# facebookresearch/pytorchvideo

Measured on NVIDIA H100. Metric: clips/sec forward (synthetic 3xTx224^2), higher is better.
Workload: dtype f16

## Files before the change

### include/pv_b200.h

```cpp
#ifndef PV_B200_H_
#define PV_B200_H_

#include <stdint.h>

#ifdef __cplusplus
extern "C" {
#endif

#define PV_ABI_VERSION 1

typedef enum pv_status {
  PV_OK = 0,
  PV_ERR_INVALID = -1,
  PV_ERR_CUDA = -2,
  PV_ERR_UNSUPPORTED = -3,
  PV_ERR_NO_DEVICE = -4
} pv_status;

typedef enum pv_dtype { PV_F16 = 0, PV_F32 = 1, PV_U8 = 2, PV_I64 = 3  } pv_dtype;

typedef enum pv_act {
  PV_ACT_NONE = 0,
  PV_ACT_RELU = 1,
  PV_ACT_SWISH = 2,
  PV_ACT_GELU = 3,
  PV_ACT_SIGMOID = 4,
  PV_ACT_HSWISH = 5
} pv_act;

typedef enum pv_conv_algo {
  PV_ALGO_AUTO = 0,
  PV_ALGO_DIRECT = 1,
  PV_ALGO_TCGEN05 = 2
} pv_conv_algo;

typedef enum pv_pool_mode { PV_POOL_MAX = 0, PV_POOL_AVG = 1 } pv_pool_mode;

int pv_abi_version(void);
const char* pv_last_error(void);
int pv_device_info(int* sm_count, int* cc);
long long pv_launch_count(void);
int pv_kernel_counts(char* buf, int len);

typedef struct pv_clip_transform_desc {
  int C, n_t, out_h, out_w;
  long long sc, st, sh, sw;
  float mean[4], stdv[4];
  int src_dtype;
  int dst_dtype;
  int div255;
} pv_clip_transform_desc;

int pv_clip_transform_fwd(const pv_clip_transform_desc* d, const void* src,
                          const int32_t* idx_t,
                          const int32_t* y0, const int32_t* y1, const float* ly,
                          const int32_t* x0, const int32_t* x1, const float* lx,
                          void* dst, void* stream);

typedef struct pv_clip_batch_desc {
  int C, n_clips, n_t, n_slow;
  int in_h, in_w, new_h, new_w;
  int top, left, out_h, out_w;
  int hflip;
  long long sc, st, sh, sw, s_clip;
  long long d_clip, d_slow_clip;
  float mean[4], stdv[4];
  int div255, normalize;
  int src_dtype, dst_dtype;
} pv_clip_batch_desc;

int pv_clip_transform_batch(const pv_clip_batch_desc* d, const void* src, const int32_t* idx_t,
                            const int32_t* slow_pos, const int32_t* geom, void* dst, void* dst_slow,
                            void* stream);

int pv_clip_transform_rrc(const pv_clip_batch_desc* d, const void* src, const int32_t* idx_t, const int32_t* boxes,
                          void* dst, void* stream);

#define PV_BOX_F32 1
#define PV_BOX_F64 3
#define PV_BOX_CLIP_SRC 1
#define PV_BOX_SCALE 2
#define PV_BOX_CROP 4
#define PV_BOX_CLIP_CROP 8
#define PV_BOX_FLIP 16
#define PV_BOX_CLIP_OUT 32
#define PV_BOX_ALL_STEPS 63

typedef struct pv_boxes_desc {
  int n_clips, n_boxes;
  int steps;
  int dtype;
  int in_h, in_w;
  int new_h, new_w, top, left, hflip;
  int out_h, out_w;
} pv_boxes_desc;

int pv_clip_boxes_transform(const pv_boxes_desc* d, const void* boxes_in, const int32_t* box_start,
                            const int32_t* geom, void* boxes_out, float* rois_out, void* stream);

typedef enum pv_aug_kind {
  PV_AUG_NONE = 0, PV_AUG_BRIGHTNESS = 1, PV_AUG_CONTRAST = 2, PV_AUG_SATURATION = 3, PV_AUG_SHARPNESS = 4,
  PV_AUG_AUTOCONTRAST = 5, PV_AUG_EQUALIZE = 6, PV_AUG_INVERT = 7, PV_AUG_POSTERIZE = 8, PV_AUG_SOLARIZE = 9,
  PV_AUG_AFFINE = 10
} pv_aug_kind;

typedef struct pv_aug_op {
  int kind;
  int ival;
  float ratio;
  float omr;
  float theta[6];
  float fill[3];
} pv_aug_op;

typedef struct pv_aug_frame_stats {
  float mn[3], mx[3];
  double gray_sum;
  unsigned char lut[3][256];
} pv_aug_frame_stats;

typedef struct pv_augment_desc {
  int n_clips, src_div, T, C, H, W;
  long long s_clip, st, sc, sh, sw;
  int dtype;
} pv_augment_desc;

int pv_augment_stats(const pv_augment_desc* d, const void* src, pv_aug_frame_stats* stats, void* stream);
int pv_augment_apply(const pv_augment_desc* d, const void* src, const pv_aug_op* ops, const pv_aug_frame_stats* stats,
                     void* dst, void* stream);
int pv_augment_mix(const pv_augment_desc* d, const void* src, const void* chains, int width, const float* mix,
                   void* dst, void* stream);

typedef struct pv_mix_desc {
  int B;
  int dtype;
  long long size[4];
  long long stride[4];
  long long s_batch;
} pv_mix_desc;

typedef struct pv_mix_label_desc {
  int B, K;
  int one_hot;
  int mode;
  float lam, oml;
  float on, off;
  long long s_row, s_col;
} pv_mix_label_desc;

int pv_mixup(const pv_mix_desc* d, void* x, float lam, float oml, void* stream);
int pv_cutmix(const pv_mix_desc* d, void* x, int yl, int yh, int xl, int xh, void* stream);
int pv_mix_labels(const pv_mix_label_desc* d, const void* labels, void* out, int* flag, void* stream);

int pv_view_reduce(const float* preds, float* out, int n_videos, int n_views, int K, int mode, void* stream);

int pv_ncdhw_to_ndhwc(const void* src, int src_dtype, void* dst, int dst_dtype,
                      int N, int C, int T, int H, int W, int c_pad, long long dst_row_stride,
                      void* stream);
int pv_ncdhw_to_ndhwc_padw(const void* src, int src_dtype, void* dst, int dst_dtype,
                           int N, int C, int T, int H, int W, int c_pad, int w_pad, int w_phys,
                           void* stream);
int pv_zero_f32(float* dst, long long n, void* stream);
int pv_ndhwc_to_ncdhw(const void* src, int src_dtype, long long src_row_stride, float* dst,
                      int N, int C, int T, int H, int W, void* stream);

typedef struct pv_conv3d_desc {
  int dtype;
  int N, Ti, Hi, Wi, Ci;
  int To, Ho, Wo, Co;
  int kt, kh, kw;
  int st, sh, sw;
  int pt, ph, pw;
  int dt, dh, dw;
  int groups;
  int act;
  int has_residual;
  long long x_row_stride, y_row_stride, res_row_stride;
  int ci_pad64;
  int x_w_pad, x_w_phys;
  long long x_batch_stride, y_batch_stride;
  const void* addend;
  long long add_n_stride, add_t_stride;
  int add_ch_off;
  const float* pre_scale;
  const float* pre_bias;
  int pre_act;
} pv_conv3d_desc;

int pv_temporal_tap_sum(const void* yk, void* y, int dtype, int N, int Ti, int To, long long hw, int Co,
                        int kt, int st, int pt, int dil, const float* scale, const float* bias, int act,
                        long long in_row_stride, long long out_row_stride, void* stream);

int pv_conv3d_fwd(const pv_conv3d_desc* d, int algo, const void* x, const void* w,
                  const float* scale, const float* bias, const void* residual, void* y,
                  void* stream);
int pv_dwconv3d_fwd(const pv_conv3d_desc* d, const void* x, const void* w, const float* scale,
                    const float* bias, void* y, float* se_sums, void* stream);
int pv_dwplane_supported(const pv_conv3d_desc* d);
int pv_dwplane_fwd(const pv_conv3d_desc* d, const void* x, const void* w, const float* scale,
                   const float* bias, void* y, void* stream);

int pv_conv3d_tcgen05_supported(const pv_conv3d_desc* d);
int pv_conv3d_group_span(const pv_conv3d_desc* d, int* span_groups, int* span_k, int* span_n);

int pv_conv3d_stem_rows_supported(const pv_conv3d_desc* d);
int pv_conv3d_stem_rows_fwd(const pv_conv3d_desc* d, const void* x, const void* w, const float* scale,
                            const float* bias, const void* zero_row, void* y, void* stream);

int pv_conv3d_stem_stream_supported(const pv_conv3d_desc* d);
int pv_conv3d_stem_stream_fwd(const pv_conv3d_desc* d, const void* x, const void* w, const float* scale,
                              const float* bias, const void* zero_row, void* y, void* stream);

typedef struct pv_bottleneck_desc {
  int N, T, H, W;
  int Cin, Cmid, Cout;
  int kt, sb;
  int has_shortcut;
  int act;
  long long x_row_stride, y_row_stride;
} pv_bottleneck_desc;
int pv_bottleneck_fused_supported(const pv_bottleneck_desc* d);
int pv_bottleneck_fused_fwd(const pv_bottleneck_desc* d, const void* x, const void* wa, const void* wb,
                            const void* wc, const void* wsc, const float* sa, const float* ba,
                            const float* sb, const float* bb, const float* sc, const float* bc,
                            const float* ssc, const float* bsc, void* y, void* stream);
int pv_bottleneck_fused_tiling(const pv_bottleneck_desc* d, int sm_count, int* tile_h, int* tile_w,
                               int* frames_per_cta, long long* smem_bytes);

typedef struct pv_pool3d_desc {
  int dtype, mode;
  int N, Ti, Hi, Wi, C;
  int To, Ho, Wo;
  int kt, kh, kw, st, sh, sw, pt, ph, pw;
  long long x_row_stride, y_row_stride;
  long long x_batch_stride, y_batch_stride;
} pv_pool3d_desc;
int pv_pool3d_fwd(const pv_pool3d_desc* d, const void* x, void* y, void* stream);

int pv_channel_sum(const void* x, int dtype, long long row_stride, int N, long long npos, int C,
                   float* sums, void* stream);
int pv_se_gate(const float* sums, long long npos, int N, int C, int Cr,
               const float* w1, const float* b1, const float* w2, const float* b2,
               int c_stride_w, float* gate, void* stream);
int pv_scale_act(const void* x, void* y, int dtype, long long x_row_stride,
                 long long y_row_stride, int N, long long npos, int C, const float* gate,
                 int act, void* stream);

int pv_roi_align_fwd(const void* x, int dtype, long long x_row_stride, int N, int H, int W, int C,
                     const float* rois, int K, int pooled_h, int pooled_w, float spatial_scale,
                     int sampling_ratio, void* y, long long y_row_stride, void* stream);

int pv_head_reduce(const void* x, int dtype, long long row_stride, int N, long long npos,
                   int C_valid, int softmax, float* out, void* stream);

int pv_layernorm(const void* x, void* y, int dtype, long long rows, int groups, int C,
                 long long x_row_stride, long long y_row_stride, const float* gamma,
                 const float* beta, float eps, void* stream);
int pv_layernorm_sets(const void* x, void* y, int dtype, long long rows, int groups, int C,
                      long long x_row_stride, long long y_row_stride, const float* gamma, const float* beta,
                      int groups_per_set, const void* cls_src, long long cls_batch_stride, long long npos,
                      float eps, void* stream);
int pv_copy_rows(const void* src, void* dst, int dtype, long long rows, int C,
                 long long src_row_stride, long long dst_row_stride, void* stream);
int pv_add_pos_cls(const void* x, void* y, int dtype, int B, long long n_patch, int C,
                   long long x_row_stride, const float* pos, int has_cls, void* stream);
int pv_add_pos_cls_to(const void* x, int x_dtype, void* y, int y_dtype, int B, long long n_patch, int C,
                      long long x_row_stride, const float* pos, int has_cls, void* stream);
int pv_add_layernorm(const void* a, int a_dtype, long long a_row_stride, const void* b, long long b_row_stride,
                     float* sum, long long sum_row_stride, void* y, long long y_row_stride, long long rows, int C,
                     const float* gamma, const float* beta, float eps, void* stream);
typedef struct pv_attention_desc {
  int dtype;
  int B, H, Nq, Nk, D;
  long long q_row_stride, k_row_stride, v_row_stride, o_row_stride;
  long long q_batch_stride, k_batch_stride, v_batch_stride, o_batch_stride;
  float scale;
  int add_q_residual;
  int normalize;
} pv_attention_desc;
int pv_attention_fwd(const pv_attention_desc* d, const void* q, const void* k, const void* v,
                     void* o, void* stream);
typedef enum pv_attention_kernel {
  PV_ATTN_WGMMA = 1,
  PV_ATTN_MMA = 2,
  PV_ATTN_SIMT = 3,
  PV_ATTN_WIDE = 4
} pv_attention_kernel;
int pv_attention_kernel_for(const pv_attention_desc* d, const void* q, const void* k, const void* v, const void* o);
int pv_attention_masked_fwd(const pv_attention_desc* d, const void* q, const void* k, const void* v, void* o,
                            const unsigned char* key_valid, float* lse_out, void* stream);
int pv_attention_weights(const pv_attention_desc* d, const void* q, const void* k, const unsigned char* key_valid,
                         const float* lse, float* w, void* stream);

int pv_masked_pool(const void* x, int dtype, long long x_row_stride, int B, int T, int C, const unsigned char* mask,
                   int mode, void* y, long long y_row_stride, void* stream);
int pv_masked_default(const void* x, int dtype, long long x_row_stride, int B, int C, const unsigned char* mask, int T,
                      const float* def, void* y, long long y_row_stride, void* stream);
int pv_mask_force_first(const unsigned char* src, unsigned char* dst, int B, int T, void* stream);
int pv_reduce_fusion(const void* const* xs, const long long* x_row_strides, int P, int dtype, long long rows, int C,
                     int op, void* y, long long y_row_stride, void* stream);
int pv_lstm_recurrence(const void* G, int dtype, long long g_row_stride, const float* w_hh_t, const unsigned char* mask,
                       int B, int T, int H, int ndir, void* y, long long y_row_stride, void* stream);

int pv_rows_l2_normalize(const void* x, int dtype, long long x_row_stride, float* y, long long y_row_stride, int rows,
                         int C, void* stream);
int pv_contrastive_ce(const float* q, long long q_row_stride, const float* k, long long k_row_stride, int N, int M, int C,
                      float temperature, long long row_offset, int mode, float* row_loss, float* loss, void* stream);
int pv_memory_bank_ce(const float* x, long long x_row_stride, const float* memory, long long bank_rows, int dim,
                      const long long* idx, int B, int K1, float temperature, float* logits, float* row_loss, float* loss,
                      int* flag, void* stream);
int pv_soft_target_ce(const void* x, int x_dtype, long long x_row_stride, const void* target, int t_dtype,
                      long long t_row_stride, int N, int C, int normalize, float eps, int reduce_mean, float* row_loss,
                      float* loss, void* stream);
int pv_ema_update(float* const* dst, const float* const* src, const long long* numel, const long long* chunks,
                  int n_chunks, float mmt, float one_minus_mmt, void* stream);
int pv_weights_refresh(const long long* gather_jobs, const long long* gather_chunks, int n_gather_chunks, const int* map,
                       const float* const* srcs, const long long* fold_jobs, int n_fold_jobs, void* stream);

int pv_bank_workspace(int op, int N, long long M, int k, long long* bytes);
int pv_bank_topk(const float* q, long long q_row_stride, int N, const float* memory, long long M, int dim, int k,
                 const long long* labels, int n_classes, float temperature, void* workspace, long long workspace_bytes,
                 float* sim_out, long long* idx_out, float* preds, int* flag, void* stream);
int pv_bank_update(const float* x, long long x_row_stride, int N, const long long* ind, float* memory, long long M,
                   int dim, float momentum, float one_minus_momentum, int* flag, void* stream);
int pv_queue_ce(const float* q, long long q_row_stride, int N, int dim, const float* queue, long long K,
                const float* keys, long long key_row_stride, int n_views, int skip_view, const float* logits,
                long long logits_row_stride, int L, float temperature, void* workspace, long long workspace_bytes,
                int reduce_mean, float* row_loss, float* loss, void* stream);

#define PV_CJ_BLUR_PASSES 3

typedef struct pv_cj_view {
  int clip;
  int n_ops;
  int ops[4];
  float factor[3];
  int hue_shift;
  int gray;
  int blur_r;
  unsigned int blur_ww, blur_fw;
} pv_cj_view;

typedef struct pv_colorjitter_desc {
  int n_views, n_t, H, W;
  long long s_clip, sc, st, sh, sw;
  int src_dtype;
  int src_scale;
} pv_colorjitter_desc;

int pv_colorjitter_stats(const pv_colorjitter_desc* d, const void* src, const int32_t* frame_idx,
                         const pv_cj_view* views, unsigned long long* sums, void* stream);
int pv_colorjitter_apply(const pv_colorjitter_desc* d, const void* src, const int32_t* frame_idx,
                         const pv_cj_view* views, const unsigned long long* sums, uint8_t* dst, void* stream);
int pv_colorjitter_vblur(const pv_colorjitter_desc* d, const pv_cj_view* views, uint8_t* dst, void* stream);

#ifdef __cplusplus
}
#endif
#endif
```

### pytorchvideo_b200/_lib.py

```python
import ctypes as C
import os

from . import _build

PV_F16, PV_F32, PV_U8, PV_I64 = 0, 1, 2, 3
ACT_NONE, ACT_RELU, ACT_SWISH, ACT_GELU, ACT_SIGMOID, ACT_HSWISH = 0, 1, 2, 3, 4, 5
ALGO_AUTO, ALGO_DIRECT, ALGO_TCGEN05 = 0, 1, 2
POOL_MAX, POOL_AVG = 0, 1
MPOOL_MAX, MPOOL_AVG, MPOOL_SUM = 0, 1, 2
REDUCE_MAX, REDUCE_SUM, REDUCE_PROD = 0, 1, 2
ATTN_WGMMA, ATTN_MMA, ATTN_SIMT, ATTN_WIDE = 1, 2, 3, 4

c_ll = C.c_longlong
c_vp = C.c_void_p


class ClipTransformDesc(C.Structure):
    _fields_ = [("C", C.c_int), ("n_t", C.c_int), ("out_h", C.c_int), ("out_w", C.c_int),
                ("sc", c_ll), ("st", c_ll), ("sh", c_ll), ("sw", c_ll),
                ("mean", C.c_float * 4), ("stdv", C.c_float * 4),
                ("src_dtype", C.c_int), ("dst_dtype", C.c_int), ("div255", C.c_int)]


class ClipBatchDesc(C.Structure):
    _fields_ = [("C", C.c_int), ("n_clips", C.c_int), ("n_t", C.c_int), ("n_slow", C.c_int),
                ("in_h", C.c_int), ("in_w", C.c_int), ("new_h", C.c_int), ("new_w", C.c_int),
                ("top", C.c_int), ("left", C.c_int), ("out_h", C.c_int), ("out_w", C.c_int),
                ("hflip", C.c_int),
                ("sc", c_ll), ("st", c_ll), ("sh", c_ll), ("sw", c_ll), ("s_clip", c_ll),
                ("d_clip", c_ll), ("d_slow_clip", c_ll),
                ("mean", C.c_float * 4), ("stdv", C.c_float * 4),
                ("div255", C.c_int), ("normalize", C.c_int), ("src_dtype", C.c_int), ("dst_dtype", C.c_int)]


BOX_F32, BOX_F64 = 1, 3
BOX_CLIP_SRC, BOX_SCALE, BOX_CROP, BOX_CLIP_CROP, BOX_FLIP, BOX_CLIP_OUT = 1, 2, 4, 8, 16, 32


class BoxesDesc(C.Structure):
    _fields_ = [("n_clips", C.c_int), ("n_boxes", C.c_int), ("steps", C.c_int), ("dtype", C.c_int),
                ("in_h", C.c_int), ("in_w", C.c_int), ("new_h", C.c_int), ("new_w", C.c_int),
                ("top", C.c_int), ("left", C.c_int), ("hflip", C.c_int), ("out_h", C.c_int), ("out_w", C.c_int)]


class AugOp(C.Structure):
    _fields_ = [("kind", C.c_int), ("ival", C.c_int), ("ratio", C.c_float), ("omr", C.c_float),
                ("theta", C.c_float * 6), ("fill", C.c_float * 3)]


class AugFrameStats(C.Structure):
    _fields_ = [("mn", C.c_float * 3), ("mx", C.c_float * 3), ("gray_sum", C.c_double), ("lut", (C.c_ubyte * 256) * 3)]


class AugmentDesc(C.Structure):
    _fields_ = [("n_clips", C.c_int), ("src_div", C.c_int), ("T", C.c_int), ("C", C.c_int), ("H", C.c_int),
                ("W", C.c_int), ("s_clip", c_ll), ("st", c_ll), ("sc", c_ll), ("sh", c_ll), ("sw", c_ll),
                ("dtype", C.c_int)]


class MixDesc(C.Structure):
    _fields_ = [("B", C.c_int), ("dtype", C.c_int), ("size", c_ll * 4), ("stride", c_ll * 4), ("s_batch", c_ll)]


class MixLabelDesc(C.Structure):
    _fields_ = [("B", C.c_int), ("K", C.c_int), ("one_hot", C.c_int), ("mode", C.c_int),
                ("lam", C.c_float), ("oml", C.c_float), ("on", C.c_float), ("off", C.c_float),
                ("s_row", c_ll), ("s_col", c_ll)]


class CjView(C.Structure):
    _fields_ = [("clip", C.c_int), ("n_ops", C.c_int), ("ops", C.c_int * 4), ("factor", C.c_float * 3),
                ("hue_shift", C.c_int), ("gray", C.c_int), ("blur_r", C.c_int), ("blur_ww", C.c_uint),
                ("blur_fw", C.c_uint)]


class ColorJitterDesc(C.Structure):
    _fields_ = [("n_views", C.c_int), ("n_t", C.c_int), ("H", C.c_int), ("W", C.c_int),
                ("s_clip", c_ll), ("sc", c_ll), ("st", c_ll), ("sh", c_ll), ("sw", c_ll),
                ("src_dtype", C.c_int), ("src_scale", C.c_int)]


class BottleneckDesc(C.Structure):
    _fields_ = [("N", C.c_int), ("T", C.c_int), ("H", C.c_int), ("W", C.c_int),
                ("Cin", C.c_int), ("Cmid", C.c_int), ("Cout", C.c_int), ("kt", C.c_int), ("sb", C.c_int),
                ("has_shortcut", C.c_int), ("act", C.c_int), ("x_row_stride", c_ll), ("y_row_stride", c_ll)]


class Conv3dDesc(C.Structure):
    _fields_ = [("dtype", C.c_int),
                ("N", C.c_int), ("Ti", C.c_int), ("Hi", C.c_int), ("Wi", C.c_int), ("Ci", C.c_int),
                ("To", C.c_int), ("Ho", C.c_int), ("Wo", C.c_int), ("Co", C.c_int),
                ("kt", C.c_int), ("kh", C.c_int), ("kw", C.c_int),
                ("st", C.c_int), ("sh", C.c_int), ("sw", C.c_int),
                ("pt", C.c_int), ("ph", C.c_int), ("pw", C.c_int),
                ("dt", C.c_int), ("dh", C.c_int), ("dw", C.c_int),
                ("groups", C.c_int), ("act", C.c_int), ("has_residual", C.c_int),
                ("x_row_stride", c_ll), ("y_row_stride", c_ll), ("res_row_stride", c_ll),
                ("ci_pad64", C.c_int), ("x_w_pad", C.c_int), ("x_w_phys", C.c_int),
                ("x_batch_stride", c_ll), ("y_batch_stride", c_ll),
                ("addend", c_vp), ("add_n_stride", c_ll), ("add_t_stride", c_ll), ("add_ch_off", C.c_int),
                ("pre_scale", c_vp), ("pre_bias", c_vp), ("pre_act", C.c_int)]


class Pool3dDesc(C.Structure):
    _fields_ = [("dtype", C.c_int), ("mode", C.c_int),
                ("N", C.c_int), ("Ti", C.c_int), ("Hi", C.c_int), ("Wi", C.c_int), ("C", C.c_int),
                ("To", C.c_int), ("Ho", C.c_int), ("Wo", C.c_int),
                ("kt", C.c_int), ("kh", C.c_int), ("kw", C.c_int),
                ("st", C.c_int), ("sh", C.c_int), ("sw", C.c_int),
                ("pt", C.c_int), ("ph", C.c_int), ("pw", C.c_int),
                ("x_row_stride", c_ll), ("y_row_stride", c_ll),
                ("x_batch_stride", c_ll), ("y_batch_stride", c_ll)]


class AttentionDesc(C.Structure):
    _fields_ = [("dtype", C.c_int), ("B", C.c_int), ("H", C.c_int), ("Nq", C.c_int),
                ("Nk", C.c_int), ("D", C.c_int),
                ("q_row_stride", c_ll), ("k_row_stride", c_ll), ("v_row_stride", c_ll),
                ("o_row_stride", c_ll),
                ("q_batch_stride", c_ll), ("k_batch_stride", c_ll), ("v_batch_stride", c_ll),
                ("o_batch_stride", c_ll),
                ("scale", C.c_float), ("add_q_residual", C.c_int), ("normalize", C.c_int)]


SIGNATURES = {
    "pv_abi_version": (C.c_int, []),
    "pv_last_error": (C.c_char_p, []),
    "pv_device_info": (C.c_int, [C.POINTER(C.c_int), C.POINTER(C.c_int)]),
    "pv_launch_count": (c_ll, []),
    "pv_kernel_counts": (C.c_int, [C.c_char_p, C.c_int]),
    "pv_clip_transform_fwd": (C.c_int, [C.POINTER(ClipTransformDesc), c_vp, c_vp, c_vp, c_vp, c_vp,
                                        c_vp, c_vp, c_vp, c_vp, c_vp]),
    "pv_clip_transform_batch": (C.c_int, [C.POINTER(ClipBatchDesc), c_vp, c_vp, c_vp, c_vp, c_vp, c_vp, c_vp]),
    "pv_clip_transform_rrc": (C.c_int, [C.POINTER(ClipBatchDesc), c_vp, c_vp, c_vp, c_vp, c_vp]),
    "pv_clip_boxes_transform": (C.c_int, [C.POINTER(BoxesDesc), c_vp, c_vp, c_vp, c_vp, c_vp, c_vp]),
    "pv_augment_stats": (C.c_int, [C.POINTER(AugmentDesc), c_vp, c_vp, c_vp]),
    "pv_augment_apply": (C.c_int, [C.POINTER(AugmentDesc), c_vp, c_vp, c_vp, c_vp, c_vp]),
    "pv_augment_mix": (C.c_int, [C.POINTER(AugmentDesc), c_vp, c_vp, C.c_int, c_vp, c_vp, c_vp]),
    "pv_mixup": (C.c_int, [C.POINTER(MixDesc), c_vp, C.c_float, C.c_float, c_vp]),
    "pv_cutmix": (C.c_int, [C.POINTER(MixDesc), c_vp, C.c_int, C.c_int, C.c_int, C.c_int, c_vp]),
    "pv_mix_labels": (C.c_int, [C.POINTER(MixLabelDesc), c_vp, c_vp, c_vp, c_vp]),
    "pv_view_reduce": (C.c_int, [c_vp, c_vp, C.c_int, C.c_int, C.c_int, C.c_int, c_vp]),
    "pv_ncdhw_to_ndhwc": (C.c_int, [c_vp, C.c_int, c_vp, C.c_int, C.c_int, C.c_int, C.c_int,
                                    C.c_int, C.c_int, C.c_int, c_ll, c_vp]),
    "pv_ncdhw_to_ndhwc_padw": (C.c_int, [c_vp, C.c_int, c_vp, C.c_int, C.c_int, C.c_int, C.c_int,
                                         C.c_int, C.c_int, C.c_int, C.c_int, C.c_int, c_vp]),
    "pv_zero_f32": (C.c_int, [c_vp, c_ll, c_vp]),
    "pv_ndhwc_to_ncdhw": (C.c_int, [c_vp, C.c_int, c_ll, c_vp, C.c_int, C.c_int, C.c_int,
                                    C.c_int, C.c_int, c_vp]),
    "pv_conv3d_fwd": (C.c_int, [C.POINTER(Conv3dDesc), C.c_int, c_vp, c_vp, c_vp, c_vp, c_vp,
                                c_vp, c_vp]),
    "pv_dwconv3d_fwd": (C.c_int, [C.POINTER(Conv3dDesc), c_vp, c_vp, c_vp, c_vp, c_vp, c_vp, c_vp]),
    "pv_dwplane_supported": (C.c_int, [C.POINTER(Conv3dDesc)]),
    "pv_dwplane_fwd": (C.c_int, [C.POINTER(Conv3dDesc), c_vp, c_vp, c_vp, c_vp, c_vp, c_vp]),
    "pv_temporal_tap_sum": (C.c_int, [c_vp, c_vp, C.c_int, C.c_int, C.c_int, C.c_int, c_ll, C.c_int, C.c_int,
                                      C.c_int, C.c_int, C.c_int, c_vp, c_vp, C.c_int, c_ll, c_ll, c_vp]),
    "pv_conv3d_tcgen05_supported": (C.c_int, [C.POINTER(Conv3dDesc)]),
    "pv_conv3d_group_span": (C.c_int, [C.POINTER(Conv3dDesc), C.POINTER(C.c_int), C.POINTER(C.c_int), C.POINTER(C.c_int)]),
    "pv_conv3d_stem_rows_supported": (C.c_int, [C.POINTER(Conv3dDesc)]),
    "pv_conv3d_stem_rows_fwd": (C.c_int, [C.POINTER(Conv3dDesc), c_vp, c_vp, c_vp, c_vp, c_vp, c_vp, c_vp]),
    "pv_conv3d_stem_stream_supported": (C.c_int, [C.POINTER(Conv3dDesc)]),
    "pv_conv3d_stem_stream_fwd": (C.c_int, [C.POINTER(Conv3dDesc), c_vp, c_vp, c_vp, c_vp, c_vp, c_vp, c_vp]),
    "pv_bottleneck_fused_supported": (C.c_int, [C.POINTER(BottleneckDesc)]),
    "pv_bottleneck_fused_fwd": (C.c_int, [C.POINTER(BottleneckDesc)] + [c_vp] * 15),
    "pv_bottleneck_fused_tiling": (C.c_int, [C.POINTER(BottleneckDesc), C.c_int, C.POINTER(C.c_int), C.POINTER(C.c_int),
                                             C.POINTER(C.c_int), C.POINTER(c_ll)]),
    "pv_pool3d_fwd": (C.c_int, [C.POINTER(Pool3dDesc), c_vp, c_vp, c_vp]),
    "pv_channel_sum": (C.c_int, [c_vp, C.c_int, c_ll, C.c_int, c_ll, C.c_int, c_vp, c_vp]),
    "pv_se_gate": (C.c_int, [c_vp, c_ll, C.c_int, C.c_int, C.c_int, c_vp, c_vp, c_vp, c_vp,
                             C.c_int, c_vp, c_vp]),
    "pv_scale_act": (C.c_int, [c_vp, c_vp, C.c_int, c_ll, c_ll, C.c_int, c_ll, C.c_int, c_vp,
                               C.c_int, c_vp]),
    "pv_head_reduce": (C.c_int, [c_vp, C.c_int, c_ll, C.c_int, c_ll, C.c_int, C.c_int, c_vp,
                                 c_vp]),
    "pv_roi_align_fwd": (C.c_int, [c_vp, C.c_int, c_ll, C.c_int, C.c_int, C.c_int, C.c_int, c_vp, C.c_int, C.c_int,
                                   C.c_int, C.c_float, C.c_int, c_vp, c_ll, c_vp]),
    "pv_layernorm": (C.c_int, [c_vp, c_vp, C.c_int, c_ll, C.c_int, C.c_int, c_ll, c_ll, c_vp, c_vp,
                               C.c_float, c_vp]),
    "pv_layernorm_sets": (C.c_int, [c_vp, c_vp, C.c_int, c_ll, C.c_int, C.c_int, c_ll, c_ll, c_vp, c_vp, C.c_int, c_vp,
                                    c_ll, c_ll, C.c_float, c_vp]),
    "pv_copy_rows": (C.c_int, [c_vp, c_vp, C.c_int, c_ll, C.c_int, c_ll, c_ll, c_vp]),
    "pv_add_pos_cls": (C.c_int, [c_vp, c_vp, C.c_int, C.c_int, c_ll, C.c_int, c_ll, c_vp, C.c_int, c_vp]),
    "pv_add_pos_cls_to": (C.c_int, [c_vp, C.c_int, c_vp, C.c_int, C.c_int, c_ll, C.c_int, c_ll, c_vp, C.c_int, c_vp]),
    "pv_add_layernorm": (C.c_int, [c_vp, C.c_int, c_ll, c_vp, c_ll, c_vp, c_ll, c_vp, c_ll, c_ll, C.c_int, c_vp, c_vp,
                                   C.c_float, c_vp]),
    "pv_attention_fwd": (C.c_int, [C.POINTER(AttentionDesc), c_vp, c_vp, c_vp, c_vp, c_vp]),
    "pv_attention_kernel_for": (C.c_int, [C.POINTER(AttentionDesc), c_vp, c_vp, c_vp, c_vp]),
    "pv_attention_masked_fwd": (C.c_int, [C.POINTER(AttentionDesc), c_vp, c_vp, c_vp, c_vp, c_vp, c_vp, c_vp]),
    "pv_attention_weights": (C.c_int, [C.POINTER(AttentionDesc), c_vp, c_vp, c_vp, c_vp, c_vp, c_vp]),
    "pv_masked_pool": (C.c_int, [c_vp, C.c_int, c_ll, C.c_int, C.c_int, C.c_int, c_vp, C.c_int, c_vp, c_ll, c_vp]),
    "pv_masked_default": (C.c_int, [c_vp, C.c_int, c_ll, C.c_int, C.c_int, c_vp, C.c_int, c_vp, c_vp, c_ll, c_vp]),
    "pv_mask_force_first": (C.c_int, [c_vp, c_vp, C.c_int, C.c_int, c_vp]),
    "pv_reduce_fusion": (C.c_int, [c_vp, c_vp, C.c_int, C.c_int, c_ll, C.c_int, C.c_int, c_vp, c_ll, c_vp]),
    "pv_lstm_recurrence": (C.c_int, [c_vp, C.c_int, c_ll, c_vp, c_vp, C.c_int, C.c_int, C.c_int, C.c_int, c_vp, c_ll,
                                     c_vp]),
    "pv_rows_l2_normalize": (C.c_int, [c_vp, C.c_int, c_ll, c_vp, c_ll, C.c_int, C.c_int, c_vp]),
    "pv_contrastive_ce": (C.c_int, [c_vp, c_ll, c_vp, c_ll, C.c_int, C.c_int, C.c_int, C.c_float, c_ll, C.c_int, c_vp,
                                    c_vp, c_vp]),
    "pv_memory_bank_ce": (C.c_int, [c_vp, c_ll, c_vp, c_ll, C.c_int, c_vp, C.c_int, C.c_int, C.c_float, c_vp, c_vp, c_vp,
                                    c_vp, c_vp]),
    "pv_soft_target_ce": (C.c_int, [c_vp, C.c_int, c_ll, c_vp, C.c_int, c_ll, C.c_int, C.c_int, C.c_int, C.c_float,
                                    C.c_int, c_vp, c_vp, c_vp]),
    "pv_ema_update": (C.c_int, [c_vp, c_vp, c_vp, c_vp, C.c_int, C.c_float, C.c_float, c_vp]),
    "pv_weights_refresh": (C.c_int, [c_vp, c_vp, C.c_int, c_vp, c_vp, c_vp, C.c_int, c_vp]),
    "pv_colorjitter_stats": (C.c_int, [C.POINTER(ColorJitterDesc), c_vp, c_vp, c_vp, c_vp, c_vp]),
    "pv_colorjitter_apply": (C.c_int, [C.POINTER(ColorJitterDesc), c_vp, c_vp, c_vp, c_vp, c_vp, c_vp]),
    "pv_colorjitter_vblur": (C.c_int, [C.POINTER(ColorJitterDesc), c_vp, c_vp, c_vp]),
    "pv_bank_workspace": (C.c_int, [C.c_int, C.c_int, c_ll, C.c_int, C.POINTER(c_ll)]),
    "pv_bank_topk": (C.c_int, [c_vp, c_ll, C.c_int, c_vp, c_ll, C.c_int, C.c_int, c_vp, C.c_int, C.c_float, c_vp, c_ll,
                               c_vp, c_vp, c_vp, c_vp, c_vp]),
    "pv_bank_update": (C.c_int, [c_vp, c_ll, C.c_int, c_vp, c_vp, c_ll, C.c_int, C.c_float, C.c_float, c_vp, c_vp]),
    "pv_queue_ce": (C.c_int, [c_vp, c_ll, C.c_int, C.c_int, c_vp, c_ll, c_vp, c_ll, C.c_int, C.c_int, c_vp, c_ll,
                              C.c_int, C.c_float, c_vp, c_ll, C.c_int, c_vp, c_vp, c_vp]),
}

_lib = None


def lib_path():
    return _build.LIB_PATH


def load():
    global _lib
    if _lib is not None:
        return _lib
    path = _build.LIB_PATH
    if not os.path.exists(path) or _build.needs_build():
        path = _build.build()
    lib = C.CDLL(path)
    for name, (res, args) in SIGNATURES.items():
        fn = getattr(lib, name)
        fn.restype = res
        fn.argtypes = args
    if lib.pv_abi_version() != 1:
        raise RuntimeError("libpvb200 ABI version mismatch")
    _lib = lib
    return lib


def last_error():
    return load().pv_last_error().decode("utf-8", "replace")


def check(rc, what=""):
    if rc != 0:
        raise RuntimeError("libpvb200 %s failed (status %d): %s" % (what, rc, last_error()))


def require_device():
    sm, cc = C.c_int(0), C.c_int(0)
    rc = load().pv_device_info(C.byref(sm), C.byref(cc))
    check(rc, "pv_device_info")
    return sm.value, cc.value


def launch_count():
    return int(load().pv_launch_count())


def group_span(desc):
    sg, sk, sn = C.c_int(0), C.c_int(0), C.c_int(0)
    ok = load().pv_conv3d_group_span(C.byref(desc), C.byref(sg), C.byref(sk), C.byref(sn))
    return bool(ok), sg.value, sk.value, sn.value


def kernel_counts():
    lib = load()
    n = lib.pv_kernel_counts(None, 0)
    while True:
        buf = C.create_string_buffer(n + 1)
        m = lib.pv_kernel_counts(buf, n + 1)
        if m <= n:
            break
        n = m
    out = {}
    for line in buf.value.decode().splitlines():
        name, count = line.rsplit(" ", 1)
        out[name] = int(count)
    return out
```

### pytorchvideo_b200/csrc/pv_stem_stream.cu

```cuda
#include "pv_common.cuh"
#include "pv_sm90.cuh"
#include "pv_epilogue.cuh"

#include <stdlib.h>
#include <string.h>

namespace pv {

using namespace sm90;

typedef CUresult (*EncodeTiledFn)(CUtensorMap*, CUtensorMapDataType, cuuint32_t, void*,
                                  const cuuint64_t*, const cuuint64_t*, const cuuint32_t*,
                                  const cuuint32_t*, CUtensorMapInterleave, CUtensorMapSwizzle,
                                  CUtensorMapL2promotion, CUtensorMapFloatOOBfill);
EncodeTiledFn get_encode_fn();

constexpr int SS_CONS_WARPS = 8;
constexpr int SS_PROD_WARPS = 3;
constexpr int SS_THREADS = (SS_CONS_WARPS + SS_PROD_WARPS + 1) * 32;
constexpr int SS_DMA_WARP = SS_CONS_WARPS + SS_PROD_WARPS;
constexpr int SS_CO = 8;

struct StreamParams {
  int N, Ti, Hi, To, Ho;
  int kh, sh, pt, ph, dh;
  int win;
  int wtiles;
  int stages;
  unsigned seg_bytes;
  unsigned w_bytes;
  long long row_pitch;
  long long base_off;
  EpiParams epi;
};

template <int KT, int KS>
__global__ void __launch_bounds__(SS_THREADS, 1)
conv3d_stem_stream_kernel(const __grid_constant__ StreamParams P, const unsigned char* __restrict__ x,
                          const unsigned char* __restrict__ w, const unsigned char* __restrict__ zero_row,
                          const float* __restrict__ scale, const float* __restrict__ bias) {
  constexpr int BN = KT * SS_CO;
  extern __shared__ uint8_t smem_raw[];
  const uint32_t smem_base = (smem_u32(smem_raw) + 1023u) & ~1023u;
  uint8_t* smem_gen = smem_raw + (smem_base - smem_u32(smem_raw));
  const int stages = P.stages;
  const uint32_t ring_off = (P.w_bytes + 1023u) & ~1023u;
  const uint32_t stage_bytes = (uint32_t)P.kh * P.seg_bytes + 2048u;
  const uint32_t staging_off = (ring_off + (uint32_t)stages * stage_bytes + 1023u) & ~1023u;
  const uint32_t staging = smem_base + staging_off;
  const uint32_t bar_base = staging + (uint32_t)(P.epi.nbuf * EPI_STAGING_BYTES);
  auto full_bar = [&](int s) { return bar_base + 8u * s; };
  auto empty_bar = [&](int s) { return bar_base + 8u * (stages + s); };
  const EpiSmem epi{staging, smem_gen + staging_off, bar_base + 8u * (2 * stages)};
  const uint32_t w_bar = epi.bars + 8u * EPI_BARS;

  const int warp = threadIdx.x >> 5, lane = threadIdx.x & 31;
  if (threadIdx.x == 0) {
    for (int s = 0; s < stages; ++s) { mbar_init(full_bar(s), 1); mbar_init(empty_bar(s), SS_CONS_WARPS); }
    epi.init();
    mbar_init(w_bar, 1);
    prefetch_tmap(&P.epi.y_map);
    fence_mbar_init();
  }
  __syncthreads();
  asm volatile("griddepcontrol.wait;" ::: "memory");
  asm volatile("griddepcontrol.launch_dependents;" ::: "memory");

  const int units = P.N * P.Ho * P.wtiles;
  auto unit_coords = [&](int u, int& wt, int& ho, int& n) {
    wt = u % P.wtiles; u /= P.wtiles;
    ho = u % P.Ho; n = u / P.Ho;
  };

  if (warp == SS_DMA_WARP) {
    if (!elect_one()) return;
    const int my_units = blockIdx.x < units ? (units - 1 - (int)blockIdx.x) / (int)gridDim.x + 1 : 0;
    const long long my_tiles = (long long)my_units * P.To;
    for (int b = 0; b < P.epi.nbuf; ++b)
      if (b < my_tiles) mbar_arrive(epi.ready(b));
    int b = 0;
    uint32_t phase = 0;
    long long k = 0;
    for (int u = blockIdx.x; u < units; u += gridDim.x) {
      int wt, ho, n;
      unit_coords(u, wt, ho, n);
      for (int to = 0; to < P.To; ++to, ++k) {
        mbar_wait(epi.full(b), phase);
        tma_store_5d(&P.epi.y_map, epi.buf(b), 0, wt * 128, ho, to, n);
        tma_store_commit();
        tma_store_wait_read0();
        if (k + P.epi.nbuf < my_tiles) mbar_arrive(epi.ready(b));
        if (++b == P.epi.nbuf) { b = 0; phase ^= 1u; }
      }
    }
    tma_store_wait_all();
  } else if (warp >= SS_CONS_WARPS) {
    const int pw = warp - SS_CONS_WARPS;
    if (pw == 0 && elect_one()) {
      mbar_arrive_expect_tx(w_bar, P.w_bytes);
      for (uint32_t o = 0; o < P.w_bytes; o += 32768u)
        bulk_g2s(smem_base + o, w + o, min(32768u, P.w_bytes - o), w_bar);
    }
    int stage = 0;
    uint32_t phase = 0;
    const long long frame_pitch = P.row_pitch * P.Hi;
    for (int u = blockIdx.x; u < units; u += gridDim.x) {
      int wt, ho, n;
      unit_coords(u, wt, ho, n);
      const long long col0 = P.base_off + (long long)wt * 128 * 16;
      long long want = 127ll * 16 + (long long)P.win * 2;
      if (col0 + want > P.row_pitch) want = P.row_pitch - col0;
      const uint32_t nbytes = (uint32_t)want;
      for (int ti = 0; ti < P.Ti; ++ti) {
        mbar_wait(empty_bar(stage), phase ^ 1u);
        const uint32_t st_base = smem_base + ring_off + (uint32_t)stage * stage_bytes;
        if (elect_one()) {
          if (pw == 0) mbar_arrive_expect_tx(full_bar(stage), (uint32_t)P.kh * nbytes);
          const unsigned char* frame = x + ((long long)n * P.Ti + ti) * frame_pitch + col0;
          for (int r = pw; r < P.kh; r += SS_PROD_WARPS) {
            const int hi = ho * P.sh - P.ph + r * P.dh;
            const unsigned char* src = (unsigned)hi < (unsigned)P.Hi ? frame + (long long)hi * P.row_pitch : zero_row;
            bulk_g2s(st_base + (uint32_t)r * P.seg_bytes, src, nbytes, full_bar(stage));
          }
        }
        __syncwarp();
        if (++stage == stages) { stage = 0; phase ^= 1u; }
      }
    }
  } else {
    const int ctid = threadIdx.x;
    const uint32_t a_row_off = (uint32_t)(ctid >> 7) * 64u * 16u;
    constexpr uint32_t b_lbo = (uint32_t)BN * 16u;
    int stage = 0, rstage = 0, epi_buf = 0;
    uint32_t phase = 0, epi_phase = 0;
    float acc[BN / 2];
    float ring[KT][4];
    float frag[8];
#pragma unroll
    for (int i = 0; i < BN / 2; ++i) acc[i] = 0.f;
#pragma unroll
    for (int i = 4; i < 8; ++i) frag[i] = 0.f;
    mbar_wait(w_bar, 0);
    auto finish = [&](const float (&v)[4], int to, int wt, int ho, int n) {
#pragma unroll
      for (int i = 0; i < 4; ++i) frag[i] = v[i];
      epilogue_tile<16>(P.epi, epi, epi_buf, epi_phase, scale, bias, frag, ctid, 0, wt * 128, ho, to, n);
    };
    auto issue = [&](float (&a)[BN / 2]) {
      mbar_wait(full_bar(stage), phase);
      const uint32_t st_base = smem_base + ring_off + (uint32_t)stage * stage_bytes;
      acc_fence(a);
      wgmma_fence();
#pragma unroll 1
      for (int r = 0; r < P.kh; ++r) {
#pragma unroll
        for (int ks = 0; ks < KS; ++ks) {
          const uint64_t a_desc = make_noswz_desc(st_base + (uint32_t)r * P.seg_bytes + (uint32_t)ks * 32u + a_row_off, 16u, 128u);
          const uint64_t b_desc = make_noswz_desc(smem_base + (uint32_t)((r * P.win + ks * 16) >> 3) * b_lbo, b_lbo, 128u);
          Wgmma<BN>::mma(a, a_desc, b_desc, (r | ks) != 0 ? 1u : 0u);
        }
      }
      wgmma_commit();
      acc_fence(a);
      if (++stage == stages) { stage = 0; phase ^= 1u; }
    };
    auto retire = [&](float (&a)[BN / 2], int ti, int wt, int ho, int n) {
      acc_fence(a);
      mbar_arrive_if(empty_bar(rstage), lane == 0);
      if (++rstage == stages) rstage = 0;
#pragma unroll
      for (int j = 0; j < KT; ++j)
#pragma unroll
        for (int i = 0; i < 4; ++i) ring[j][i] += a[4 * j + i];
      const int done = ti + P.pt - (KT - 1);
      if ((unsigned)done < (unsigned)P.To) finish(ring[KT - 1], done, wt, ho, n);
#pragma unroll
      for (int s = KT - 1; s > 0; --s)
#pragma unroll
        for (int i = 0; i < 4; ++i) ring[s][i] = ring[s - 1][i];
#pragma unroll
      for (int i = 0; i < 4; ++i) ring[0][i] = 0.f;
    };
    for (int u = blockIdx.x; u < units; u += gridDim.x) {
      int wt, ho, n;
      unit_coords(u, wt, ho, n);
#pragma unroll
      for (int s = 0; s < KT; ++s)
#pragma unroll
        for (int i = 0; i < 4; ++i) ring[s][i] = 0.f;
#pragma unroll 1
      for (int ti = 0; ti < P.Ti; ++ti) {
        issue(acc);
        wgmma_wait<0>();
        retire(acc, ti, wt, ho, n);
      }
#pragma unroll
      for (int s = KT - 1; s > 0; --s) {
        const int to = P.Ti - 1 + P.pt - (s - 1);
        if ((unsigned)to < (unsigned)P.To) finish(ring[s], to, wt, ho, n);
      }
    }
  }
}

static int stream_window_lead(const pv_conv3d_desc* d) { return (((d->x_w_pad - d->pw) * d->Ci * 2) % 16) ? 1 : 0; }

}

using namespace pv;

extern "C" int pv_conv3d_stem_stream_supported(const pv_conv3d_desc* d) {
  if (!d || d->dtype != PV_F16 || d->groups != 1 || d->has_residual || d->addend || !act_known(d->act)) return 0;
  if (conv3d_has_prologue(d)) return 0;
  if (d->Ci != 4 || d->sw != 2 || d->dw != 1 || d->x_w_pad <= 0 || d->x_row_stride != 4) return 0;
  if (d->x_w_pad < d->pw || (d->x_w_phys * 8) % 16) return 0;
  if (d->Co != SS_CO || d->kt != 5 || d->st != 1 || d->dt != 1 || d->pt < 0 || d->pt >= d->kt) return 0;
  if (d->To != d->Ti + 2 * d->pt - (d->kt - 1) || d->To <= 0 || d->Ti <= 0) return 0;
  if (d->kh < 1 || d->kh > 16 || d->y_row_stride % 8) return 0;
  const int lead = stream_window_lead(d);
  const int run = (d->kw + lead) * 4;
  const int win = run <= 16 ? 16 : (run <= 32 ? 32 : 64);
  if (win != 32 || d->ci_pad64 != win) return 0;
  const long long base_off = (long long)(d->x_w_pad - d->pw - lead) * 8;
  if (base_off < 0 || base_off % 16) return 0;
  if (base_off + (long long)(d->Wo - 1) * 16 + (long long)win * 2 > (long long)d->x_w_phys * 8) return 0;
  return 1;
}

extern "C" int pv_conv3d_stem_stream_fwd(const pv_conv3d_desc* d, const void* x, const void* w, const float* scale,
                                         const float* bias, const void* zero_row, void* y, void* stream) {
  PV_CHECK_ARG(d && x && w && scale && bias && zero_row && y, "null argument");
  if (!pv_conv3d_stem_stream_supported(d)) { set_error("stem stream kernel: unsupported convolution"); return PV_ERR_UNSUPPORTED; }
  EncodeTiledFn encode = get_encode_fn();
  if (!encode) { set_error("cuTensorMapEncodeTiled entry point unavailable"); return PV_ERR_CUDA; }
  const int sm_count = current_sm_count();
  if (sm_count <= 0) { set_error("cannot query the SM count"); return PV_ERR_CUDA; }
  StreamParams P;
  memset(&P, 0, sizeof(P));
  P.N = d->N; P.Ti = d->Ti; P.Hi = d->Hi; P.To = d->To; P.Ho = d->Ho;
  P.kh = d->kh; P.sh = d->sh; P.pt = d->pt; P.ph = d->ph; P.dh = d->dh;
  P.win = d->ci_pad64;
  P.wtiles = (int)cdiv(d->Wo, 128);
  P.row_pitch = (long long)d->x_w_phys * 8;
  P.base_off = (long long)(d->x_w_pad - d->pw - stream_window_lead(d)) * 8;
  P.w_bytes = (unsigned)((long long)d->kh * P.win * d->kt * SS_CO * 2);
  P.seg_bytes = (unsigned)((127 * 16 + P.win * 2 + 127) & ~127);
  const unsigned stage_bytes = (unsigned)P.kh * P.seg_bytes + 2048u;
  P.epi.nbuf = EPI_MAX_BUFS;
  const size_t smem_fixed = 2048 + ((P.w_bytes + 1023) & ~1023u) + 1024 + epi_smem_bytes(P.epi.nbuf) + 8 * (2 * 8 + 1) + 16;
  {
    long long st = (227 * 1024 - (long long)smem_fixed) / stage_bytes;
    if (st > 8) st = 8;
    if (st < 2) { set_error("stem stream kernel: not enough shared memory for two stages"); return PV_ERR_UNSUPPORTED; }
    P.stages = (int)st;
  }
  const size_t smem_bytes = smem_fixed + (size_t)P.stages * stage_bytes;
  P.epi.block_n = 16;
  P.epi.Co = d->Co;
  P.epi.rows = d->Wo < 128 ? d->Wo : 128;
  P.epi.act = d->act;
  P.epi.has_residual = 0;
  epi_set_addend(P.epi, d);
  const long long ostr[4] = {1, d->Wo, (long long)d->Wo * d->Ho, (long long)d->Wo * d->Ho * d->To};
  const int O[4] = {d->Wo, d->Ho, d->To, d->N};
  const int box[4] = {P.epi.rows, 1, 1, 1};
  for (int m = 0; m < 4; ++m) {
    P.epi.o_ext[m] = O[m];
    P.epi.o_box[m] = box[m];
    P.epi.o_pos[m] = (int)ostr[m];
  }
  {
    cuuint64_t gdim[5] = {(cuuint64_t)d->Co, (cuuint64_t)O[0], (cuuint64_t)O[1], (cuuint64_t)O[2], (cuuint64_t)O[3]};
    cuuint64_t gstr[4];
    cuuint32_t bx[5] = {64, (cuuint32_t)box[0], 1, 1, 1}, estr[5] = {1, 1, 1, 1, 1};
    for (int m = 0; m < 4; ++m) gstr[m] = (cuuint64_t)(ostr[m] * d->y_row_stride * 2);
    CUresult cr = encode(&P.epi.y_map, CU_TENSOR_MAP_DATA_TYPE_FLOAT16, 5, y, gdim, gstr, bx, estr, CU_TENSOR_MAP_INTERLEAVE_NONE,
                         CU_TENSOR_MAP_SWIZZLE_128B, CU_TENSOR_MAP_L2_PROMOTION_L2_128B, CU_TENSOR_MAP_FLOAT_OOB_FILL_NONE);
    if (cr != CUDA_SUCCESS) { set_error("cuTensorMapEncodeTiled(stem stream Y) failed: %d", (int)cr); return PV_ERR_CUDA; }
  }
  const long long units = (long long)d->N * d->Ho * P.wtiles;
  if (units == 0) return PV_OK;
  PV_CHECK_ARG(units * d->To < (1ll << 31), "too many tiles");
  const int grid = (int)(units < sm_count ? units : sm_count);
  cudaLaunchConfig_t cfg;
  memset(&cfg, 0, sizeof(cfg));
  cfg.gridDim = dim3((unsigned)grid);
  cfg.blockDim = dim3(SS_THREADS);
  cfg.dynamicSmemBytes = smem_bytes;
  cfg.stream = (cudaStream_t)stream;
  cudaLaunchAttribute attr[1];
  attr[0].id = cudaLaunchAttributeProgrammaticStreamSerialization;
  attr[0].val.programmaticStreamSerializationAllowed = 1;
  cfg.attrs = attr;
  cfg.numAttrs = 1;
  const unsigned char *xb = (const unsigned char*)x, *wb = (const unsigned char*)w, *zb = (const unsigned char*)zero_row;
  const char* name = nullptr;
#define PV_SS_LAUNCH(KT, KS)                                                                              \
  if (d->kt == KT && P.win == 16 * KS) {                                                                  \
    PV_OPT_IN_SMEM((conv3d_stem_stream_kernel<KT, KS>), 227 * 1024);                                      \
    PV_CUDA_OK(cudaLaunchKernelEx(&cfg, conv3d_stem_stream_kernel<KT, KS>, P, xb, wb, zb, scale, bias));  \
    name = "conv3d_stem_stream_kernel<" #KT "," #KS ">";                                                   \
  }
  PV_SS_LAUNCH(5, 2)
#undef PV_SS_LAUNCH
  if (!name) { set_error("internal: no stem stream instance for kt=%d win=%d", d->kt, P.win); return PV_ERR_INVALID; }
  PV_LAUNCH_OK(name);
  return PV_OK;
}
```

Before: 2096.

## Run two stem-stream CTAs per SM by shrinking epilogue staging and stages

Reworks shared-memory planning for the stem stream conv kernel so it targets two resident CTAs per SM. To fit, it uses a single epilogue staging buffer with a trimmed tail and recomputes the pipeline stage count from half the SM's shared memory. The launch grid is now sized from the queried occupancy times the SM count rather than one CTA per SM, and launch bounds are raised to 2. The aim is to hide producer/consumer and epilogue latency across CTAs, at the cost of fewer pipeline stages, fewer epilogue buffers and a tighter register budget per thread.

```diff
diff --git a/include/pv_b200.h b/include/pv_b200.h
--- a/include/pv_b200.h
+++ b/include/pv_b200.h
@@ -210,6 +210,11 @@
 int pv_conv3d_stem_stream_supported(const pv_conv3d_desc* d);
 int pv_conv3d_stem_stream_fwd(const pv_conv3d_desc* d, const void* x, const void* w, const float* scale,
                               const float* bias, const void* zero_row, void* y, void* stream);
+int pv_conv3d_stem_stream_tiling(const pv_conv3d_desc* d, int sm_count, int max_ctas_per_sm, int* ctas_per_sm,
+                                 int* stages, int* nbuf, int* grid, long long* smem_bytes);
+int pv_conv3d_stem_stream_fwd_ctas(const pv_conv3d_desc* d, const void* x, const void* w, const float* scale,
+                                   const float* bias, const void* zero_row, void* y, int max_ctas_per_sm,
+                                   int* ctas_per_sm, void* stream);
 
 typedef struct pv_bottleneck_desc {
   int N, T, H, W;
diff --git a/pytorchvideo_b200/_lib.py b/pytorchvideo_b200/_lib.py
--- a/pytorchvideo_b200/_lib.py
+++ b/pytorchvideo_b200/_lib.py
@@ -161,6 +161,11 @@
     "pv_conv3d_stem_rows_fwd": (C.c_int, [C.POINTER(Conv3dDesc), c_vp, c_vp, c_vp, c_vp, c_vp, c_vp, c_vp]),
     "pv_conv3d_stem_stream_supported": (C.c_int, [C.POINTER(Conv3dDesc)]),
     "pv_conv3d_stem_stream_fwd": (C.c_int, [C.POINTER(Conv3dDesc), c_vp, c_vp, c_vp, c_vp, c_vp, c_vp, c_vp]),
+    "pv_conv3d_stem_stream_tiling": (C.c_int, [C.POINTER(Conv3dDesc), C.c_int, C.c_int, C.POINTER(C.c_int),
+                                               C.POINTER(C.c_int), C.POINTER(C.c_int), C.POINTER(C.c_int),
+                                               C.POINTER(c_ll)]),
+    "pv_conv3d_stem_stream_fwd_ctas": (C.c_int, [C.POINTER(Conv3dDesc), c_vp, c_vp, c_vp, c_vp, c_vp, c_vp, C.c_int,
+                                                 C.POINTER(C.c_int), c_vp]),
     "pv_bottleneck_fused_supported": (C.c_int, [C.POINTER(BottleneckDesc)]),
     "pv_bottleneck_fused_fwd": (C.c_int, [C.POINTER(BottleneckDesc)] + [c_vp] * 15),
     "pv_bottleneck_fused_tiling": (C.c_int, [C.POINTER(BottleneckDesc), C.c_int, C.POINTER(C.c_int), C.POINTER(C.c_int),
diff --git a/pytorchvideo_b200/csrc/pv_stem_stream.cu b/pytorchvideo_b200/csrc/pv_stem_stream.cu
--- a/pytorchvideo_b200/csrc/pv_stem_stream.cu
+++ b/pytorchvideo_b200/csrc/pv_stem_stream.cu
@@ -20,6 +20,9 @@
 constexpr int SS_THREADS = (SS_CONS_WARPS + SS_PROD_WARPS + 1) * 32;
 constexpr int SS_DMA_WARP = SS_CONS_WARPS + SS_PROD_WARPS;
 constexpr int SS_CO = 8;
+constexpr int SS_STAGING_TAIL = 128 * 128;
+constexpr int SS_SM_SMEM = 228 * 1024;
+constexpr int SS_CTA_RESERVED = 1024;
 
 struct StreamParams {
   int N, Ti, Hi, To, Ho;
@@ -35,7 +38,7 @@
 };
 
 template <int KT, int KS>
-__global__ void __launch_bounds__(SS_THREADS, 1)
+__global__ void __launch_bounds__(SS_THREADS, 2)
 conv3d_stem_stream_kernel(const __grid_constant__ StreamParams P, const unsigned char* __restrict__ x,
                           const unsigned char* __restrict__ w, const unsigned char* __restrict__ zero_row,
                           const float* __restrict__ scale, const float* __restrict__ bias) {
@@ -48,7 +51,7 @@
   const uint32_t stage_bytes = (uint32_t)P.kh * P.seg_bytes + 2048u;
   const uint32_t staging_off = (ring_off + (uint32_t)stages * stage_bytes + 1023u) & ~1023u;
   const uint32_t staging = smem_base + staging_off;
-  const uint32_t bar_base = staging + (uint32_t)(P.epi.nbuf * EPI_STAGING_BYTES);
+  const uint32_t bar_base = staging + (uint32_t)((P.epi.nbuf - 1) * EPI_STAGING_BYTES + SS_STAGING_TAIL);
   auto full_bar = [&](int s) { return bar_base + 8u * s; };
   auto empty_bar = [&](int s) { return bar_base + 8u * (stages + s); };
   const EpiSmem epi{staging, smem_gen + staging_off, bar_base + 8u * (2 * stages)};
@@ -227,15 +230,8 @@
   return 1;
 }
 
-extern "C" int pv_conv3d_stem_stream_fwd(const pv_conv3d_desc* d, const void* x, const void* w, const float* scale,
-                                         const float* bias, const void* zero_row, void* y, void* stream) {
-  PV_CHECK_ARG(d && x && w && scale && bias && zero_row && y, "null argument");
-  if (!pv_conv3d_stem_stream_supported(d)) { set_error("stem stream kernel: unsupported convolution"); return PV_ERR_UNSUPPORTED; }
-  EncodeTiledFn encode = get_encode_fn();
-  if (!encode) { set_error("cuTensorMapEncodeTiled entry point unavailable"); return PV_ERR_CUDA; }
-  const int sm_count = current_sm_count();
-  if (sm_count <= 0) { set_error("cannot query the SM count"); return PV_ERR_CUDA; }
-  StreamParams P;
+namespace {
+int stream_plan(const pv_conv3d_desc* d, int max_ctas_per_sm, StreamParams& P, int& ctas_per_sm, size_t& smem_bytes) {
   memset(&P, 0, sizeof(P));
   P.N = d->N; P.Ti = d->Ti; P.Hi = d->Hi; P.To = d->To; P.Ho = d->Ho;
   P.kh = d->kh; P.sh = d->sh; P.pt = d->pt; P.ph = d->ph; P.dh = d->dh;
@@ -245,22 +241,92 @@
   P.base_off = (long long)(d->x_w_pad - d->pw - stream_window_lead(d)) * 8;
   P.w_bytes = (unsigned)((long long)d->kh * P.win * d->kt * SS_CO * 2);
   P.seg_bytes = (unsigned)((127 * 16 + P.win * 2 + 127) & ~127);
-  const unsigned stage_bytes = (unsigned)P.kh * P.seg_bytes + 2048u;
-  P.epi.nbuf = EPI_MAX_BUFS;
-  const size_t smem_fixed = 2048 + ((P.w_bytes + 1023) & ~1023u) + 1024 + epi_smem_bytes(P.epi.nbuf) + 8 * (2 * 8 + 1) + 16;
-  {
-    long long st = (227 * 1024 - (long long)smem_fixed) / stage_bytes;
-    if (st > 8) st = 8;
-    if (st < 2) { set_error("stem stream kernel: not enough shared memory for two stages"); return PV_ERR_UNSUPPORTED; }
-    P.stages = (int)st;
-  }
-  const size_t smem_bytes = smem_fixed + (size_t)P.stages * stage_bytes;
   P.epi.block_n = 16;
   P.epi.Co = d->Co;
   P.epi.rows = d->Wo < 128 ? d->Wo : 128;
   P.epi.act = d->act;
   P.epi.has_residual = 0;
   epi_set_addend(P.epi, d);
+  const unsigned stage_bytes = (unsigned)P.kh * P.seg_bytes + 2048u;
+  for (int ctas = 2; ctas >= 1; --ctas) {
+    if (max_ctas_per_sm > 0 && ctas > max_ctas_per_sm) continue;
+    const int nbuf = ctas == 2 ? 1 : EPI_MAX_BUFS;
+    const size_t smem_fixed = 2048 + ((P.w_bytes + 1023) & ~1023u) + 1024 + (size_t)(nbuf - 1) * EPI_STAGING_BYTES +
+                              SS_STAGING_TAIL + 8 * EPI_BARS + 8 * (2 * 8 + 1) + 16;
+    long long st = ((long long)SS_SM_SMEM / ctas - SS_CTA_RESERVED - (long long)smem_fixed) / stage_bytes;
+    if (st > 8) st = 8;
+    if (st < 2) continue;
+    P.stages = (int)st;
+    P.epi.nbuf = nbuf;
+    ctas_per_sm = ctas;
+    smem_bytes = smem_fixed + (size_t)P.stages * stage_bytes;
+    return PV_OK;
+  }
+  set_error("stem stream kernel: not enough shared memory for two stages");
+  return PV_ERR_UNSUPPORTED;
+}
+
+template <int KT, int KS>
+int stream_occupancy(size_t smem_bytes, int& occ) {
+  static DeviceOnce once;
+  static size_t memo_smem[64];
+  static int memo_occ[64];
+  const int dev = current_device();
+  if (once.first(dev)) {
+    PV_CUDA_OK(cudaFuncSetAttribute(conv3d_stem_stream_kernel<KT, KS>, cudaFuncAttributeMaxDynamicSharedMemorySize,
+                                    227 * 1024));
+    PV_CUDA_OK(cudaFuncSetAttribute(conv3d_stem_stream_kernel<KT, KS>, cudaFuncAttributePreferredSharedMemoryCarveout,
+                                    (int)cudaSharedmemCarveoutMaxShared));
+  }
+  if (dev >= 0 && dev < 64 && memo_smem[dev] == smem_bytes) {
+    occ = memo_occ[dev];
+    return PV_OK;
+  }
+  PV_CUDA_OK(cudaOccupancyMaxActiveBlocksPerMultiprocessor(&occ, conv3d_stem_stream_kernel<KT, KS>, SS_THREADS,
+                                                           smem_bytes));
+  if (occ < 1) { set_error("stem stream kernel: no CTA of %zu shared-memory bytes fits on an SM", smem_bytes); return PV_ERR_CUDA; }
+  if (dev >= 0 && dev < 64) { memo_smem[dev] = smem_bytes; memo_occ[dev] = occ; }
+  return PV_OK;
+}
+
+long long stream_grid(long long units, int ctas_per_sm, int sm_count) {
+  const long long slots = (long long)ctas_per_sm * sm_count;
+  return units < slots ? units : slots;
+}
+}
+
+extern "C" int pv_conv3d_stem_stream_tiling(const pv_conv3d_desc* d, int sm_count, int max_ctas_per_sm,
+                                            int* ctas_per_sm, int* stages, int* nbuf, int* grid, long long* smem_bytes) {
+  PV_CHECK_ARG(d && sm_count > 0 && max_ctas_per_sm >= 0, "null descriptor, sm_count <= 0 or max_ctas_per_sm < 0");
+  if (!pv_conv3d_stem_stream_supported(d)) { set_error("stem stream kernel: unsupported convolution"); return PV_ERR_UNSUPPORTED; }
+  StreamParams P;
+  int ctas = 0;
+  size_t smem = 0;
+  const int rc = stream_plan(d, max_ctas_per_sm, P, ctas, smem);
+  if (rc != PV_OK) return rc;
+  if (ctas_per_sm) *ctas_per_sm = ctas;
+  if (stages) *stages = P.stages;
+  if (nbuf) *nbuf = P.epi.nbuf;
+  if (grid) *grid = (int)stream_grid((long long)d->N * d->Ho * P.wtiles, ctas, sm_count);
+  if (smem_bytes) *smem_bytes = (long long)smem;
+  return PV_OK;
+}
+
+extern "C" int pv_conv3d_stem_stream_fwd_ctas(const pv_conv3d_desc* d, const void* x, const void* w, const float* scale,
+                                              const float* bias, const void* zero_row, void* y, int max_ctas_per_sm,
+                                              int* ctas_per_sm, void* stream) {
+  PV_CHECK_ARG(d && x && w && scale && bias && zero_row && y, "null argument");
+  PV_CHECK_ARG(max_ctas_per_sm >= 0, "max_ctas_per_sm < 0");
+  if (!pv_conv3d_stem_stream_supported(d)) { set_error("stem stream kernel: unsupported convolution"); return PV_ERR_UNSUPPORTED; }
+  EncodeTiledFn encode = get_encode_fn();
+  if (!encode) { set_error("cuTensorMapEncodeTiled entry point unavailable"); return PV_ERR_CUDA; }
+  const int sm_count = current_sm_count();
+  if (sm_count <= 0) { set_error("cannot query the SM count"); return PV_ERR_CUDA; }
+  StreamParams P;
+  int planned = 0;
+  size_t smem_bytes = 0;
+  const int rc = stream_plan(d, max_ctas_per_sm, P, planned, smem_bytes);
+  if (rc != PV_OK) return rc;
   const long long ostr[4] = {1, d->Wo, (long long)d->Wo * d->Ho, (long long)d->Wo * d->Ho * d->To};
   const int O[4] = {d->Wo, d->Ho, d->To, d->N};
   const int box[4] = {P.epi.rows, 1, 1, 1};
@@ -281,10 +347,8 @@
   const long long units = (long long)d->N * d->Ho * P.wtiles;
   if (units == 0) return PV_OK;
   PV_CHECK_ARG(units * d->To < (1ll << 31), "too many tiles");
-  const int grid = (int)(units < sm_count ? units : sm_count);
   cudaLaunchConfig_t cfg;
   memset(&cfg, 0, sizeof(cfg));
-  cfg.gridDim = dim3((unsigned)grid);
   cfg.blockDim = dim3(SS_THREADS);
   cfg.dynamicSmemBytes = smem_bytes;
   cfg.stream = (cudaStream_t)stream;
@@ -297,7 +361,11 @@
   const char* name = nullptr;
 #define PV_SS_LAUNCH(KT, KS)                                                                              \
   if (d->kt == KT && P.win == 16 * KS) {                                                                  \
-    PV_OPT_IN_SMEM((conv3d_stem_stream_kernel<KT, KS>), 227 * 1024);                                      \
+    int occ = 0;                                                                                          \
+    const int orc = stream_occupancy<KT, KS>(smem_bytes, occ);                                            \
+    if (orc != PV_OK) return orc;                                                                         \
+    if (ctas_per_sm) *ctas_per_sm = occ;                                                                  \
+    cfg.gridDim = dim3((unsigned)stream_grid(units, occ < planned ? occ : planned, sm_count));            \
     PV_CUDA_OK(cudaLaunchKernelEx(&cfg, conv3d_stem_stream_kernel<KT, KS>, P, xb, wb, zb, scale, bias));  \
     name = "conv3d_stem_stream_kernel<" #KT "," #KS ">";                                                   \
   }
@@ -307,3 +375,8 @@
   PV_LAUNCH_OK(name);
   return PV_OK;
 }
+
+extern "C" int pv_conv3d_stem_stream_fwd(const pv_conv3d_desc* d, const void* x, const void* w, const float* scale,
+                                         const float* bias, const void* zero_row, void* y, void* stream) {
+  return pv_conv3d_stem_stream_fwd_ctas(d, x, w, scale, bias, zero_row, y, 0, nullptr, stream);
+}
```

Result: no change. 2116 (median of 6 runs) (+0.9%).
